# seungjunlee96/lightning-generative-models

Measured on AMD Instinct MI355X. Metric: training images/sec (DDPM UNet 32x32, bs=128), higher is better.
Workload: dtype f32; 1 GPU; configs/diffusion/ddpm.json UNet dim=64, 3x32x32 synthetic NCHW fp32, training_step+backward+Adam+EMA; global_batch=128, per_gpu_batch=128, parallelism=dp1, launch=hipGraph replay (1 graph/step)

## Files before the change

### lightning-generative-models_amd/csrc/linattn_fused.hip

```cpp
#include <type_traits>

#include "lgm_common.h"

namespace {

constexpr int DH = 32;
constexpr int HEADS = 4;
constexpr int HID = HEADS * DH;
constexpr int C = 64;
constexpr int LD = 36;
constexpr int TP = 128;
constexpr int XLD = 80;
constexpr int WLD = 100;

struct FArgs {
  const float* qkv;  long pitch;
  const float* gout; long gout_pitch;
  const float* ctx; const float* gctx; const float* kmax; const float* ksum; const float* rvec;
  const float* xn;   long xn_pitch;
  const float* wt;
  float* gxn;        long gxn_pitch;
  float* slabs;
  int n, tiles, items, per;
  float scale;
};

__device__ __forceinline__ void load16(const float* p, float (&v)[16]) {
#pragma unroll
  for (int q = 0; q < 4; ++q) {
    const f32x4 t = *reinterpret_cast<const f32x4*>(p + 4 * q);
    v[4 * q] = t[0]; v[4 * q + 1] = t[1]; v[4 * q + 2] = t[2]; v[4 * q + 3] = t[3];
  }
}

__global__ __launch_bounds__(256, 1) void linattn_bwd_fused_kernel(const FArgs p) {
  extern __shared__ __align__(16) float sm[];
  float* Qs = sm;
  float* Ks = Qs + TP * LD;
  float* Vs = Ks + TP * LD;
  float* Gs = Vs + TP * LD;
  float* Cs = Gs + TP * LD;
  float* GCs = Cs + DH * LD;
  float* GCt = GCs + DH * LD;
  float* rr = GCt + DH * LD;
  float* Ws = rr + DH;
  float* Xs = Ws + C * WLD;
  const int tid = threadIdx.x;
  const int lane = tid & 63, wid = tid >> 6;
  const int lr = lane & 31, lh = lane >> 5;
  const int l16 = lane & 15, lq = lane >> 4;
  const int c4 = (tid & 7) * 4, prow = tid >> 3;
  const int srow = 32 * wid + (lane >> 1), spart = (lane & 1) * 16;
  const int it0 = blockIdx.x * p.per, it1 = min(p.items, it0 + p.per);
  if (it0 >= it1) return;

  int w_src[6], w_dst[6];
#pragma unroll
  for (int u = 0; u < 6; ++u) {
    const int e = tid + 256 * u;
    const int c = e / 24, rem = e - 24 * c;
    const int part = rem >> 3, j = rem & 7;
    w_src[u] = c * (3 * HID) + part * HID + 4 * j;
    w_dst[u] = c * WLD + part * DH + 4 * j;
  }

  f32x4 q4[4], k4[4], v4[4], g4[4], km4, ks4, cx4, gc4, w4[6];
  float rr1 = 0.f;
  auto issue = [&](int it, int h) {
    const int b = it / p.tiles, i0 = (it % p.tiles) * TP;
    const int rows = min(TP, p.n - i0);
    const long bh = (long)b * HEADS + h;
#pragma unroll
    for (int u = 0; u < 4; ++u) {
      const int r = prow + 32 * u;
      const long row = (long)b * p.n + i0 + (r < rows ? r : 0);
      const float* qp = p.qkv + row * p.pitch + h * DH + c4;
      q4[u] = *reinterpret_cast<const f32x4*>(qp);
      k4[u] = *reinterpret_cast<const f32x4*>(qp + HID);
      v4[u] = *reinterpret_cast<const f32x4*>(qp + 2 * HID);
      g4[u] = *reinterpret_cast<const f32x4*>(p.gout + row * p.gout_pitch + h * DH + c4);
    }
    km4 = *reinterpret_cast<const f32x4*>(p.kmax + bh * DH + c4);
    ks4 = *reinterpret_cast<const f32x4*>(p.ksum + bh * DH + c4);
    cx4 = *reinterpret_cast<const f32x4*>(p.ctx + bh * DH * DH + tid * 4);
    gc4 = *reinterpret_cast<const f32x4*>(p.gctx + bh * DH * DH + tid * 4);
    if (tid < DH) rr1 = p.rvec[bh * DH + tid];
#pragma unroll
    for (int u = 0; u < 6; ++u) w4[u] = *reinterpret_cast<const f32x4*>(p.wt + w_src[u] + h * DH);
  };

  f32x4 dacc[HEADS][6];
#pragma unroll
  for (int h = 0; h < HEADS; ++h)
#pragma unroll
    for (int t = 0; t < 6; ++t) dacc[h][t] = f32x4{0.f, 0.f, 0.f, 0.f};
  const f32x4 zero4 = {0.f, 0.f, 0.f, 0.f};

  issue(it0, 0);
  for (int it = it0; it < it1; ++it) {
    const int b = it / p.tiles, i0 = (it % p.tiles) * TP;
    const int rows = min(TP, p.n - i0);
    f32x16 acc[2];
#pragma unroll
    for (int a = 0; a < 2; ++a)
#pragma unroll
      for (int r = 0; r < 16; ++r) acc[a][r] = 0.f;
    {
#pragma unroll
      for (int u = 0; u < 4; ++u) {
        const int r = prow + 32 * u;
        const long row = (long)b * p.n + i0 + (r < rows ? r : 0);
#pragma unroll
        for (int hf = 0; hf < 2; ++hf) {
          f32x4 xv = *reinterpret_cast<const f32x4*>(p.xn + row * p.xn_pitch + hf * 32 + c4);
          if (r >= rows) xv = zero4;
          *reinterpret_cast<f32x4*>(Xs + r * XLD + hf * 32 + c4) = xv;
        }
      }
    }
    auto head = [&](auto hc) {
      constexpr int h = decltype(hc)::value;
#pragma unroll
      for (int u = 0; u < 4; ++u) {
        const int r = prow + 32 * u;
        const bool live = r < rows;
        f32x4 kv;
#pragma unroll
        for (int k = 0; k < 4; ++k) kv[k] = __expf(k4[u][k] - km4[k]) * (1.f / ks4[k]);
        *reinterpret_cast<f32x4*>(Qs + r * LD + c4) = live ? q4[u] : zero4;
        *reinterpret_cast<f32x4*>(Ks + r * LD + c4) = live ? kv : zero4;
        *reinterpret_cast<f32x4*>(Vs + r * LD + c4) = live ? v4[u] : zero4;
        *reinterpret_cast<f32x4*>(Gs + r * LD + c4) = live ? g4[u] : zero4;
      }
      {
        const int d = tid >> 3, e0 = (tid & 7) * 4;
        *reinterpret_cast<f32x4*>(Cs + d * LD + e0) = cx4;
        *reinterpret_cast<f32x4*>(GCs + d * LD + e0) = gc4;
#pragma unroll
        for (int k = 0; k < 4; ++k) GCt[(e0 + k) * LD + d] = gc4[k];
      }
      if (tid < DH) rr[tid] = rr1;
#pragma unroll
      for (int u = 0; u < 6; ++u) *reinterpret_cast<f32x4*>(Ws + w_dst[u]) = w4[u];
      __syncthreads();
      if (h + 1 < HEADS) issue(it, h + 1);
      else if (it + 1 < it1) issue(it + 1, 0);

      float sv[16];
      {
        load16(Qs + srow * LD + spart, sv);
        float mx = sv[0];
#pragma unroll
        for (int k = 1; k < 16; ++k) mx = fmaxf(mx, sv[k]);
        mx = fmaxf(mx, __shfl_xor(mx, 1, 64));
        float sum = 0.f;
#pragma unroll
        for (int k = 0; k < 16; ++k) {
          sv[k] = __expf(sv[k] - mx);
          sum += sv[k];
        }
        sum += __shfl_xor(sum, 1, 64);
        const float inv = 1.f / sum;
#pragma unroll
        for (int k = 0; k < 16; ++k) sv[k] *= inv;
      }
      f32x16 a1, a2, a3;
#pragma unroll
      for (int r = 0; r < 16; ++r) a1[r] = a2[r] = a3[r] = 0.f;
      {
        float ca[16], ga[16], ta[16], gb[16], vb[16], kb[16];
        load16(Cs + lr * LD + 16 * lh, ca);
        load16(GCs + lr * LD + 16 * lh, ga);
        load16(GCt + lr * LD + 16 * lh, ta);
        load16(Gs + (32 * wid + lr) * LD + 16 * lh, gb);
        load16(Vs + (32 * wid + lr) * LD + 16 * lh, vb);
        load16(Ks + (32 * wid + lr) * LD + 16 * lh, kb);
#pragma unroll
        for (int s = 0; s < 16; ++s) {
          a1 = __builtin_amdgcn_mfma_f32_32x32x2f32(ca[s], gb[s], a1, 0, 0, 0);
          a2 = __builtin_amdgcn_mfma_f32_32x32x2f32(ga[s], vb[s], a2, 0, 0, 0);
          a3 = __builtin_amdgcn_mfma_f32_32x32x2f32(ta[s], kb[s], a3, 0, 0, 0);
        }
      }
      lgm_wave_lds_sync();
      {
        float* gp = Gs + (32 * wid + lr) * LD + 4 * lh;
        float* vp = Vs + (32 * wid + lr) * LD + 4 * lh;
#pragma unroll
        for (int g = 0; g < 4; ++g) {
          *reinterpret_cast<f32x4*>(gp + 8 * g) = f32x4{a1[4 * g], a1[4 * g + 1], a1[4 * g + 2], a1[4 * g + 3]};
          *reinterpret_cast<f32x4*>(vp + 8 * g) = f32x4{a2[4 * g], a2[4 * g + 1], a2[4 * g + 2], a2[4 * g + 3]};
        }
      }
      lgm_wave_lds_sync();
      {
        float g1[16], t2[16], kk[16], rv[16], dot = 0.f;
        load16(Gs + srow * LD + spart, g1);
        load16(Vs + srow * LD + spart, t2);
        load16(Ks + srow * LD + spart, kk);
        load16(rr + spart, rv);
#pragma unroll
        for (int k = 0; k < 16; ++k) {
          g1[k] *= p.scale;
          dot += sv[k] * g1[k];
        }
        dot += __shfl_xor(dot, 1, 64);
#pragma unroll
        for (int q = 0; q < 4; ++q) {
          f32x4 oq, ok;
#pragma unroll
          for (int k = 0; k < 4; ++k) {
            oq[k] = sv[4 * q + k] * (g1[4 * q + k] - dot);
            ok[k] = kk[4 * q + k] * (t2[4 * q + k] - rv[4 * q + k]);
          }
          *reinterpret_cast<f32x4*>(Qs + srow * LD + spart + 4 * q) = oq;
          *reinterpret_cast<f32x4*>(Ks + srow * LD + spart + 4 * q) = ok;
        }
      }
      lgm_wave_lds_sync();
      {
        float* vp = Vs + (32 * wid + lr) * LD + 4 * lh;
#pragma unroll
        for (int g = 0; g < 4; ++g)
          *reinterpret_cast<f32x4*>(vp + 8 * g) = f32x4{a3[4 * g], a3[4 * g + 1], a3[4 * g + 2], a3[4 * g + 3]};
      }
      lgm_wave_lds_sync();
#pragma unroll
      for (int part = 0; part < 3; ++part) {
        float xb[16], w0[16], w1[16];
        load16((part == 0 ? Qs : part == 1 ? Ks : Vs) + (32 * wid + lr) * LD + 16 * lh, xb);
        load16(Ws + lr * WLD + part * DH + 16 * lh, w0);
        load16(Ws + (32 + lr) * WLD + part * DH + 16 * lh, w1);
#pragma unroll
        for (int s = 0; s < 16; ++s) {
          acc[0] = __builtin_amdgcn_mfma_f32_32x32x2f32(w0[s], xb[s], acc[0], 0, 0, 0);
          acc[1] = __builtin_amdgcn_mfma_f32_32x32x2f32(w1[s], xb[s], acc[1], 0, 0, 0);
        }
      }
      __syncthreads();
      {
        const float* xb = Xs + lq * XLD + 16 * wid + l16;
#pragma unroll 4
        for (int s = 0; s < TP / 4; ++s) {
          const float bv = xb[4 * s * XLD];
#pragma unroll
          for (int part = 0; part < 3; ++part) {
            const float* X = (part == 0 ? Qs : part == 1 ? Ks : Vs) + (4 * s + lq) * LD + l16;
            dacc[h][2 * part] = __builtin_amdgcn_mfma_f32_16x16x4f32(X[0], bv, dacc[h][2 * part], 0, 0, 0);
            dacc[h][2 * part + 1] = __builtin_amdgcn_mfma_f32_16x16x4f32(X[16], bv, dacc[h][2 * part + 1], 0, 0, 0);
          }
        }
        __syncthreads();
      }
    };
    head(std::integral_constant<int, 0>{});
    head(std::integral_constant<int, 1>{});
    head(std::integral_constant<int, 2>{});
    head(std::integral_constant<int, 3>{});
    if (32 * wid + lr < rows) {
      float* o = p.gxn + ((long)b * p.n + i0 + 32 * wid + lr) * p.gxn_pitch + 4 * lh;
#pragma unroll
      for (int a = 0; a < 2; ++a)
#pragma unroll
        for (int g = 0; g < 4; ++g)
          *reinterpret_cast<f32x4*>(o + 32 * a + 8 * g) = f32x4{acc[a][4 * g], acc[a][4 * g + 1], acc[a][4 * g + 2], acc[a][4 * g + 3]};
    }
  }
  {
    float* sl = p.slabs + (long)blockIdx.x * (3 * HID * C);
#pragma unroll
    for (int h = 0; h < HEADS; ++h)
#pragma unroll
      for (int t = 0; t < 6; ++t)
#pragma unroll
        for (int r = 0; r < 4; ++r) {
          const int wrow = (t >> 1) * HID + h * DH + (t & 1) * 16 + 4 * lq + r;
          sl[(long)wrow * C + 16 * wid + l16] = dacc[h][t][r];
        }
  }
}

constexpr size_t kSmem = ((size_t)4 * TP * LD + 3 * DH * LD + DH + C * WLD + TP * XLD) * sizeof(float);

int plan_blocks(int B, int n, int* tiles, int* items, int* per) {
  *tiles = lgm_cdiv(n, TP);
  *items = B * *tiles;
  const int nb = *items < 256 ? *items : 256;
  *per = lgm_cdiv(*items, nb);
  return lgm_cdiv(*items, *per);
}

}

extern "C" int64_t lgm_linattn_bwd_fused_supported(int heads, int dim_head, int Cin) {
  return heads == HEADS && dim_head == DH && Cin == C ? 1 : 0;
}

extern "C" int64_t lgm_linattn_bwd_fused_slabs(int B, int n, int Cin) {
  if (Cin != C) return 0;
  int tiles, items, per;
  const int blocks = plan_blocks(B, n, &tiles, &items, &per);
  return (int64_t)blocks * 3 * HID * C * (int64_t)sizeof(float);
}

int lgm_linattn_bwd_fused_launch(const float* qkv, long pitch, const float* gout, long gout_pitch, const float* ctx,
                                 const float* gctx, const float* kmax, const float* ksum, const float* rvec,
                                 const float* xn, long xn_pitch, const float* wt, int B, int n, float scale,
                                 float* gxn, long gxn_pitch, float* slabs, int* blocks_out, hipStream_t s) {
  FArgs a;
  a.qkv = qkv; a.pitch = pitch; a.gout = gout; a.gout_pitch = gout_pitch;
  a.ctx = ctx; a.gctx = gctx; a.kmax = kmax; a.ksum = ksum; a.rvec = rvec;
  a.xn = xn; a.xn_pitch = xn_pitch; a.wt = wt; a.gxn = gxn; a.gxn_pitch = gxn_pitch;
  a.slabs = slabs; a.n = n; a.scale = scale;
  const int blocks = plan_blocks(B, n, &a.tiles, &a.items, &a.per);
  *blocks_out = blocks;
  lgm_note_kernel(LGM_KNAME("linattn_bwd_fused_kernel"));
  static bool attr = false;
  if (!attr) {
    (void)hipFuncSetAttribute(reinterpret_cast<const void*>(linattn_bwd_fused_kernel),
                              hipFuncAttributeMaxDynamicSharedMemorySize, (int)kSmem);
    attr = true;
  }
  hipLaunchKernelGGL(linattn_bwd_fused_kernel, dim3(blocks), dim3(256), kSmem, s, a);
  LGM_LAUNCH_CHECK();
  return LGM_OK;
}

namespace {

constexpr int OTP = 128;
constexpr int ALD = 132;

struct OArgs {
  const float* qkv;  long pitch;
  const float* ctx;
  const float* wout; const float* bout; const float* g;
  const float* x;    long x_pitch;
  float* ao;         long ao_pitch;
  float* o2;         long o2_pitch;
  float* y;          long y_pitch;
  int n, tiles, items, per;
  float scale;
};

template <int NC>
__global__ __launch_bounds__(256, NC == 2 ? 3 : 1) void linattn_out_fused_kernel(const OArgs p) {
  constexpr int CO = 32 * NC;
  extern __shared__ __align__(16) float sm[];
  float* Ws = sm;
  float* Ct = Ws + CO * ALD;
  const int tid = threadIdx.x;
  const int lane = tid & 63, wid = tid >> 6;
  const int lr = lane & 31, lh = lane >> 5;
  const int it0 = blockIdx.x * p.per, it1 = min(p.items, it0 + p.per);
  if (it0 >= it1) return;
  const float sqrtc = sqrtf((float)CO);

  f32x4 qn[4];
  auto issue_q = [&](int it, int h) {
    const int b = it / p.tiles, i0 = (it % p.tiles) * OTP;
    const int pix = min(i0 + 32 * wid + lr, p.n - 1);
    const float* qp = p.qkv + ((long)b * p.n + pix) * p.pitch + h * DH + 16 * lh;
#pragma unroll
    for (int j = 0; j < 4; ++j) qn[j] = *reinterpret_cast<const f32x4*>(qp + 4 * j);
  };
  issue_q(it0, 0);
#pragma unroll
  for (int u = 0; u < NC * 4; ++u) {
    const int e = tid + 256 * u;
    const int c = e >> 5, k4 = (e & 31) * 4;
    *reinterpret_cast<f32x4*>(Ws + c * ALD + k4) = *reinterpret_cast<const f32x4*>(p.wout + (long)c * HID + k4);
  }
  int b_staged = -1;
  for (int it = it0; it < it1; ++it) {
    const int b = it / p.tiles, i0 = (it % p.tiles) * OTP;
    const int pix = i0 + 32 * wid + lr;
    const bool live = pix < p.n;
    const long row = (long)b * p.n + min(pix, p.n - 1);
    if (b != b_staged) {
      __syncthreads();
#pragma unroll
      for (int u = 0; u < 4; ++u) {
        const int e = (tid + 256 * u) * 4;
        const int h = e >> 10, d = (e >> 5) & 31, e0 = e & 31;
        const f32x4 cv = *reinterpret_cast<const f32x4*>(p.ctx + (long)b * HEADS * DH * DH + e);
#pragma unroll
        for (int k = 0; k < 4; ++k) Ct[h * (DH * LD) + (e0 + k) * LD + d] = cv[k];
      }
      __syncthreads();
      b_staged = b;
    }
    f32x4 xres[NC <= 4 ? NC * 4 : 1];
    if constexpr (NC <= 4) {
#pragma unroll
      for (int a = 0; a < NC; ++a)
#pragma unroll
        for (int g = 0; g < 4; ++g)
          xres[a * 4 + g] = *reinterpret_cast<const f32x4*>(p.x + row * p.x_pitch + a * 32 + 8 * g + 4 * lh);
    }
    f32x16 acc[NC];
#pragma unroll
    for (int a = 0; a < NC; ++a)
#pragma unroll
      for (int r = 0; r < 16; ++r) acc[a][r] = 0.f;
#pragma unroll
    for (int h = 0; h < HEADS; ++h) {
      float qs[16];
#pragma unroll
      for (int j = 0; j < 4; ++j) {
        qs[4 * j] = qn[j][0]; qs[4 * j + 1] = qn[j][1]; qs[4 * j + 2] = qn[j][2]; qs[4 * j + 3] = qn[j][3];
      }
      if (h + 1 < HEADS) issue_q(it, h + 1);
      else if (it + 1 < it1) issue_q(it + 1, 0);
      float mx = qs[0];
#pragma unroll
      for (int k = 1; k < 16; ++k) mx = fmaxf(mx, qs[k]);
      mx = fmaxf(mx, __shfl_xor(mx, 32, 64));
      float sum = 0.f;
#pragma unroll
      for (int k = 0; k < 16; ++k) {
        qs[k] = __expf(qs[k] - mx);
        sum += qs[k];
      }
      sum += __shfl_xor(sum, 32, 64);
      const float inv = p.scale / sum;
      float ca[16];
      load16(Ct + h * (DH * LD) + lr * LD + 16 * lh, ca);
      f32x16 o;
#pragma unroll
      for (int r = 0; r < 16; ++r) o[r] = 0.f;
#pragma unroll
      for (int s = 0; s < 16; ++s) o = __builtin_amdgcn_mfma_f32_32x32x2f32(ca[s], qs[s] * inv, o, 0, 0, 0);
      if (live) {
#pragma unroll
        for (int g = 0; g < 4; ++g)
          *reinterpret_cast<f32x4*>(p.ao + row * p.ao_pitch + h * DH + 8 * g + 4 * lh) =
              f32x4{o[4 * g], o[4 * g + 1], o[4 * g + 2], o[4 * g + 3]};
      }
#pragma unroll
      for (int a = 0; a < NC; ++a) {
        const float* wp = Ws + (a * 32 + lr) * ALD + h * DH + 4 * lh;
#pragma unroll
        for (int g = 0; g < 4; ++g) {
          const f32x4 wv = *reinterpret_cast<const f32x4*>(wp + 8 * g);
#pragma unroll
          for (int j = 0; j < 4; ++j) acc[a] = __builtin_amdgcn_mfma_f32_32x32x2f32(wv[j], o[4 * g + j], acc[a], 0, 0, 0);
        }
      }
    }
    float ss = 0.f;
#pragma unroll
    for (int a = 0; a < NC; ++a)
#pragma unroll
      for (int g = 0; g < 4; ++g) {
        const f32x4 bv = *reinterpret_cast<const f32x4*>(p.bout + a * 32 + 8 * g + 4 * lh);
#pragma unroll
        for (int k = 0; k < 4; ++k) {
          acc[a][4 * g + k] += bv[k];
          ss += acc[a][4 * g + k] * acc[a][4 * g + k];
        }
      }
    ss += __shfl_xor(ss, 32, 64);
    const float rinv = sqrtc / fmaxf(sqrtf(ss), 1e-12f);
    if (live) {
#pragma unroll
      for (int a = 0; a < NC; ++a)
#pragma unroll
        for (int g = 0; g < 4; ++g) {
          const int c = a * 32 + 8 * g + 4 * lh;
          const f32x4 v = {acc[a][4 * g], acc[a][4 * g + 1], acc[a][4 * g + 2], acc[a][4 * g + 3]};
          const f32x4 gv = *reinterpret_cast<const f32x4*>(p.g + c);
          f32x4 xv;
          if constexpr (NC <= 4) xv = xres[a * 4 + g];
          else xv = *reinterpret_cast<const f32x4*>(p.x + row * p.x_pitch + c);
          *reinterpret_cast<f32x4*>(p.o2 + row * p.o2_pitch + c) = v;
          *reinterpret_cast<f32x4*>(p.y + row * p.y_pitch + c) = v * gv * rinv + xv;
        }
    }
  }
}

template <int NC>
int launch_out(const OArgs& a, int blocks, hipStream_t s) {
  const size_t smem = ((size_t)32 * NC * ALD + HEADS * DH * LD) * sizeof(float);
  static bool attr = false;
  if (!attr) {
    (void)hipFuncSetAttribute(reinterpret_cast<const void*>(linattn_out_fused_kernel<NC>),
                              hipFuncAttributeMaxDynamicSharedMemorySize, (int)smem);
    attr = true;
  }
  hipLaunchKernelGGL(linattn_out_fused_kernel<NC>, dim3(blocks), dim3(256), smem, s, a);
  LGM_LAUNCH_CHECK();
  return LGM_OK;
}

}

extern "C" int64_t lgm_linattn_fwd_fused_supported(int heads, int dim_head, int Cout) {
  if (heads != HEADS || dim_head != DH) return 0;
  return Cout == 64 || Cout == 128 ? 2 : Cout == 256 ? 1 : 0;
}

int lgm_linattn_out_fused_launch(const float* qkv, long pitch, const float* ctx, const float* wout, const float* bout,
                                 const float* g, const float* x, long x_pitch, float* ao, long ao_pitch, float* o2,
                                 long o2_pitch, float* y, long y_pitch, int B, int n, int Cout, float scale, hipStream_t s) {
  OArgs a;
  a.qkv = qkv; a.pitch = pitch; a.ctx = ctx; a.wout = wout; a.bout = bout; a.g = g; a.x = x; a.x_pitch = x_pitch;
  a.ao = ao; a.ao_pitch = ao_pitch; a.o2 = o2; a.o2_pitch = o2_pitch; a.y = y; a.y_pitch = y_pitch;
  a.n = n; a.scale = scale;
  a.tiles = lgm_cdiv(n, OTP);
  a.items = B * a.tiles;
  const int slots = Cout == 64 ? 768 : 256;
  const int nb = a.items < slots ? a.items : slots;
  a.per = lgm_cdiv(a.items, nb);
  const int blocks = lgm_cdiv(a.items, a.per);
  lgm_note_kernel(Cout == 64 ? LGM_KNAME("linattn_out_fused_kernel<2>") : Cout == 128 ? LGM_KNAME("linattn_out_fused_kernel<4>")
                                                                             : LGM_KNAME("linattn_out_fused_kernel<8>"));
  if (Cout == 64) return launch_out<2>(a, blocks, s);
  if (Cout == 128) return launch_out<4>(a, blocks, s);
  return launch_out<8>(a, blocks, s);
}

namespace {

struct QArgs {
  const float* x;  long x_pitch;
  const float* g;
  const float* w;
  float* xn;       long xn_pitch;
  float* qkv;      long q_pitch;
  long P;
  int items, per;
};

template <int NCI>
__global__ __launch_bounds__(256, NCI == 2 ? 3 : NCI == 4 ? 2 : 1) void rms_qkv_fused_kernel(const QArgs p) {
  constexpr int CI = 32 * NCI;
  constexpr int WL = CI + 4;
  extern __shared__ __align__(16) float sm[];
  float* Ws = sm;
  const int tid = threadIdx.x;
  const int lane = tid & 63, wid = tid >> 6;
  const int lr = lane & 31, lh = lane >> 5;
  int blk, slice;
  {
    const int nblk = (int)gridDim.x / 3, bid = (int)blockIdx.x;
    if (nblk % 8 == 0) {
      const int xcd = bid & 7, slot = bid >> 3;
      blk = (slot / 3) * 8 + xcd;
      slice = slot % 3;
    } else {
      blk = bid / 3;
      slice = bid % 3;
    }
  }
  const int it0 = blk * p.per, it1 = min(p.items, it0 + p.per);
  if (it0 >= it1) return;
  const float sqrtc = sqrtf((float)CI);
  f32x4 xr[NCI * 4];
  auto issue_x = [&](int it) {
    const long pix = (long)it * 128 + 32 * wid + lr;
    const long row = pix < p.P ? pix : p.P - 1;
#pragma unroll
    for (int a = 0; a < NCI; ++a)
#pragma unroll
      for (int g = 0; g < 4; ++g)
        xr[a * 4 + g] = *reinterpret_cast<const f32x4*>(p.x + row * p.x_pitch + a * 32 + 8 * g + 4 * lh);
  };
  issue_x(it0);
#pragma unroll
  for (int u = 0; u < NCI * 4; ++u) {
    const int e = tid + 256 * u;
    const int r = e / (CI / 4), c4 = (e % (CI / 4)) * 4;
    *reinterpret_cast<f32x4*>(Ws + r * WL + c4) = *reinterpret_cast<const f32x4*>(p.w + (long)(slice * 128 + r) * CI + c4);
  }
  __syncthreads();
  for (int it = it0; it < it1; ++it) {
    const long pix = (long)it * 128 + 32 * wid + lr;
    const bool live = pix < p.P;
    const long row = live ? pix : p.P - 1;
    f32x4 xn[NCI * 4];
    float ss = 0.f;
#pragma unroll
    for (int k = 0; k < NCI * 4; ++k) {
      xn[k] = xr[k];
      ss += xn[k][0] * xn[k][0] + xn[k][1] * xn[k][1] + xn[k][2] * xn[k][2] + xn[k][3] * xn[k][3];
    }
    if (NCI <= 4 && it + 1 < it1) issue_x(it + 1);
    ss += __shfl_xor(ss, 32, 64);
    const float inv = sqrtc / fmaxf(sqrtf(ss), 1e-12f);
#pragma unroll
    for (int a = 0; a < NCI; ++a)
#pragma unroll
      for (int g = 0; g < 4; ++g) {
        const f32x4 gv = *reinterpret_cast<const f32x4*>(p.g + a * 32 + 8 * g + 4 * lh);
        xn[a * 4 + g] = xn[a * 4 + g] * gv * inv;
        if (slice == 0 && live)
          *reinterpret_cast<f32x4*>(p.xn + row * p.xn_pitch + a * 32 + 8 * g + 4 * lh) = xn[a * 4 + g];
      }
#pragma unroll 1
    for (int t = 0; t < 4; ++t) {
      f32x16 acc;
#pragma unroll
      for (int r = 0; r < 16; ++r) acc[r] = 0.f;
      const float* wp = Ws + (t * 32 + lr) * WL + 4 * lh;
#pragma unroll
      for (int a = 0; a < NCI; ++a)
#pragma unroll
        for (int g = 0; g < 4; ++g) {
          const f32x4 wv = *reinterpret_cast<const f32x4*>(wp + a * 32 + 8 * g);
#pragma unroll
          for (int j = 0; j < 4; ++j) acc = __builtin_amdgcn_mfma_f32_32x32x2f32(wv[j], xn[a * 4 + g][j], acc, 0, 0, 0);
        }
      if (live) {
        float* o = p.qkv + row * p.q_pitch + slice * 128 + t * 32 + 4 * lh;
#pragma unroll
        for (int g = 0; g < 4; ++g)
          *reinterpret_cast<f32x4*>(o + 8 * g) = f32x4{acc[4 * g], acc[4 * g + 1], acc[4 * g + 2], acc[4 * g + 3]};
      }
    }
    if (NCI > 4 && it + 1 < it1) issue_x(it + 1);
  }
}

template <int NCI>
int launch_qkv(const QArgs& a, int blocks, hipStream_t s) {
  const size_t smem = (size_t)128 * (32 * NCI + 4) * sizeof(float);
  static bool attr = false;
  if (!attr) {
    (void)hipFuncSetAttribute(reinterpret_cast<const void*>(rms_qkv_fused_kernel<NCI>),
                              hipFuncAttributeMaxDynamicSharedMemorySize, (int)smem);
    attr = true;
  }
  hipLaunchKernelGGL(rms_qkv_fused_kernel<NCI>, dim3(blocks * 3), dim3(256), smem, s, a);
  LGM_LAUNCH_CHECK();
  return LGM_OK;
}

}

extern "C" int64_t lgm_rms_qkv_fused_supported(int C, int N) {
  if (N != 3 * HID) return 0;
  return C == 64 ? 2 : C == 128 || C == 256 ? 1 : 0;
}

extern "C" int lgm_rms_qkv_fused(const float* x, int64_t x_pitch, const float* g, const float* w, int C, int N,
                                 int64_t npix, float* xn, int64_t xn_pitch, float* qkv, int64_t qkv_pitch, void* stream) {
  LGM_REQUIRE(lgm_rms_qkv_fused_supported(C, N), "rms_qkv_fused: C=%d N=%d unsupported", C, N);
  LGM_REQUIRE(x && g && w && xn && qkv && npix > 0, "rms_qkv_fused: null pointer / empty");
  LGM_REQUIRE(x_pitch % 4 == 0 && xn_pitch % 4 == 0 && qkv_pitch % 4 == 0 && lgm_aligned16(x) && lgm_aligned16(g) &&
                  lgm_aligned16(w) && lgm_aligned16(xn) && lgm_aligned16(qkv),
              "rms_qkv_fused: 16-byte aligned operands required");
  QArgs a;
  a.x = x; a.x_pitch = x_pitch; a.g = g; a.w = w; a.xn = xn; a.xn_pitch = xn_pitch; a.qkv = qkv; a.q_pitch = qkv_pitch;
  a.P = npix;
  a.items = lgm_cdiv(npix, 128);
  const int slots = C == 64 ? 256 : C == 128 ? 170 : 85;
  const int nb = a.items < slots ? a.items : slots;
  a.per = lgm_cdiv(a.items, nb);
  const int blocks = lgm_cdiv(a.items, a.per);
  lgm_note_kernel(C == 64 ? LGM_KNAME("rms_qkv_fused_kernel<2>") : C == 128 ? LGM_KNAME("rms_qkv_fused_kernel<4>") : LGM_KNAME("rms_qkv_fused_kernel<8>"));
  hipStream_t s = (hipStream_t)stream;
  if (C == 64) return launch_qkv<2>(a, blocks, s);
  if (C == 128) return launch_qkv<4>(a, blocks, s);
  return launch_qkv<8>(a, blocks, s);
}
```

Baseline: 13680 images/s.

## Run fused linear-attention backward with 512 threads and 16x16 MFMA tiles

Measured after the change: 13780 images/s (median of 6 runs). No clear change (+0.8%).

```diff
diff --git a/lightning-generative-models_amd/csrc/linattn_fused.hip b/lightning-generative-models_amd/csrc/linattn_fused.hip
--- a/lightning-generative-models_amd/csrc/linattn_fused.hip
+++ b/lightning-generative-models_amd/csrc/linattn_fused.hip
@@ -10,7 +10,8 @@
 constexpr int C = 64;
 constexpr int LD = 36;
 constexpr int TP = 128;
-constexpr int XLD = 80;
+constexpr int BT = 512;
+constexpr int XLD = 68;
 constexpr int WLD = 100;
 
 struct FArgs {
@@ -33,7 +34,15 @@
   }
 }
 
-__global__ __launch_bounds__(256, 1) void linattn_bwd_fused_kernel(const FArgs p) {
+__device__ __forceinline__ void load8(const float* p, float (&v)[8]) {
+#pragma unroll
+  for (int q = 0; q < 2; ++q) {
+    const f32x4 t = *reinterpret_cast<const f32x4*>(p + 4 * q);
+    v[4 * q] = t[0]; v[4 * q + 1] = t[1]; v[4 * q + 2] = t[2]; v[4 * q + 3] = t[3];
+  }
+}
+
+__global__ __launch_bounds__(BT, 2) void linattn_bwd_fused_kernel(const FArgs p) {
   extern __shared__ __align__(16) float sm[];
   float* Qs = sm;
   float* Ks = Qs + TP * LD;
@@ -47,82 +56,81 @@
   float* Xs = Ws + C * WLD;
   const int tid = threadIdx.x;
   const int lane = tid & 63, wid = tid >> 6;
-  const int lr = lane & 31, lh = lane >> 5;
   const int l16 = lane & 15, lq = lane >> 4;
   const int c4 = (tid & 7) * 4, prow = tid >> 3;
-  const int srow = 32 * wid + (lane >> 1), spart = (lane & 1) * 16;
+  const int own = (16 * wid + l16) * LD + 8 * lq;
+  const int owd = (16 * wid + l16) * LD + 4 * lq;
+  const int ecg = wid & 3, erh = wid >> 2;
   const int it0 = blockIdx.x * p.per, it1 = min(p.items, it0 + p.per);
   if (it0 >= it1) return;
 
-  int w_src[6], w_dst[6];
-#pragma unroll
-  for (int u = 0; u < 6; ++u) {
-    const int e = tid + 256 * u;
-    const int c = e / 24, rem = e - 24 * c;
-    const int part = rem >> 3, j = rem & 7;
-    w_src[u] = c * (3 * HID) + part * HID + 4 * j;
-    w_dst[u] = c * WLD + part * DH + 4 * j;
-  }
-
-  f32x4 q4[4], k4[4], v4[4], g4[4], km4, ks4, cx4, gc4, w4[6];
+  const float* w_src = p.wt + prow * (3 * HID) + c4;
+  const int w_dst = prow * WLD + c4;
+
+  f32x4 q4[2], k4[2], v4[2], g4[2], km4, ks4, cg4, w4[3];
   float rr1 = 0.f;
   auto issue = [&](int it, int h) {
     const int b = it / p.tiles, i0 = (it % p.tiles) * TP;
     const int rows = min(TP, p.n - i0);
     const long bh = (long)b * HEADS + h;
-#pragma unroll
-    for (int u = 0; u < 4; ++u) {
-      const int r = prow + 32 * u;
-      const long row = (long)b * p.n + i0 + (r < rows ? r : 0);
-      const float* qp = p.qkv + row * p.pitch + h * DH + c4;
+    const float* qb = p.qkv + ((long)b * p.n + i0) * p.pitch + h * DH;
+    const float* gb = p.gout + ((long)b * p.n + i0) * p.gout_pitch + h * DH;
+#pragma unroll
+    for (int u = 0; u < 2; ++u) {
+      const int r = prow + 64 * u, rc = r < rows ? r : 0;
+      const float* qp = qb + (unsigned)(rc * (int)p.pitch + c4);
       q4[u] = *reinterpret_cast<const f32x4*>(qp);
       k4[u] = *reinterpret_cast<const f32x4*>(qp + HID);
       v4[u] = *reinterpret_cast<const f32x4*>(qp + 2 * HID);
-      g4[u] = *reinterpret_cast<const f32x4*>(p.gout + row * p.gout_pitch + h * DH + c4);
+      g4[u] = *reinterpret_cast<const f32x4*>(gb + (unsigned)(rc * (int)p.gout_pitch + c4));
     }
     km4 = *reinterpret_cast<const f32x4*>(p.kmax + bh * DH + c4);
     ks4 = *reinterpret_cast<const f32x4*>(p.ksum + bh * DH + c4);
-    cx4 = *reinterpret_cast<const f32x4*>(p.ctx + bh * DH * DH + tid * 4);
-    gc4 = *reinterpret_cast<const f32x4*>(p.gctx + bh * DH * DH + tid * 4);
+    cg4 = *reinterpret_cast<const f32x4*>((tid < 256 ? p.ctx : p.gctx) + bh * DH * DH + (tid & 255) * 4);
     if (tid < DH) rr1 = p.rvec[bh * DH + tid];
 #pragma unroll
-    for (int u = 0; u < 6; ++u) w4[u] = *reinterpret_cast<const f32x4*>(p.wt + w_src[u] + h * DH);
+    for (int u = 0; u < 3; ++u) w4[u] = *reinterpret_cast<const f32x4*>(w_src + u * HID + h * DH);
   };
 
-  f32x4 dacc[HEADS][6];
+  const f32x4 zero4 = {0.f, 0.f, 0.f, 0.f};
+  f32x4 dacc[HEADS][3];
 #pragma unroll
   for (int h = 0; h < HEADS; ++h)
 #pragma unroll
-    for (int t = 0; t < 6; ++t) dacc[h][t] = f32x4{0.f, 0.f, 0.f, 0.f};
-  const f32x4 zero4 = {0.f, 0.f, 0.f, 0.f};
+    for (int t = 0; t < 3; ++t) dacc[h][t] = zero4;
+
+  f32x4 xr[4];
+  auto issue_xn = [&](int it) {
+    const int b = it / p.tiles, i0 = (it % p.tiles) * TP;
+    const int rows = min(TP, p.n - i0);
+#pragma unroll
+    for (int u = 0; u < 2; ++u) {
+      const int r = prow + 64 * u, rc = r < rows ? r : 0;
+      const float* xp = p.xn + ((long)b * p.n + i0) * p.xn_pitch + (unsigned)(rc * (int)p.xn_pitch + c4);
+      xr[2 * u] = *reinterpret_cast<const f32x4*>(xp);
+      xr[2 * u + 1] = *reinterpret_cast<const f32x4*>(xp + 32);
+    }
+  };
 
   issue(it0, 0);
+  issue_xn(it0);
   for (int it = it0; it < it1; ++it) {
     const int b = it / p.tiles, i0 = (it % p.tiles) * TP;
     const int rows = min(TP, p.n - i0);
-    f32x16 acc[2];
-#pragma unroll
-    for (int a = 0; a < 2; ++a)
-#pragma unroll
-      for (int r = 0; r < 16; ++r) acc[a][r] = 0.f;
-    {
-#pragma unroll
-      for (int u = 0; u < 4; ++u) {
-        const int r = prow + 32 * u;
-        const long row = (long)b * p.n + i0 + (r < rows ? r : 0);
-#pragma unroll
-        for (int hf = 0; hf < 2; ++hf) {
-          f32x4 xv = *reinterpret_cast<const f32x4*>(p.xn + row * p.xn_pitch + hf * 32 + c4);
-          if (r >= rows) xv = zero4;
-          *reinterpret_cast<f32x4*>(Xs + r * XLD + hf * 32 + c4) = xv;
-        }
-      }
+    f32x4 acc[4];
+#pragma unroll
+    for (int t = 0; t < 4; ++t) acc[t] = zero4;
+#pragma unroll
+    for (int u = 0; u < 2; ++u) {
+      const int r = prow + 64 * u;
+      *reinterpret_cast<f32x4*>(Xs + r * XLD + c4) = r < rows ? xr[2 * u] : zero4;
+      *reinterpret_cast<f32x4*>(Xs + r * XLD + 32 + c4) = r < rows ? xr[2 * u + 1] : zero4;
     }
     auto head = [&](auto hc) {
       constexpr int h = decltype(hc)::value;
 #pragma unroll
-      for (int u = 0; u < 4; ++u) {
-        const int r = prow + 32 * u;
+      for (int u = 0; u < 2; ++u) {
+        const int r = prow + 64 * u;
         const bool live = r < rows;
         f32x4 kv;
 #pragma unroll
@@ -133,122 +141,141 @@
         *reinterpret_cast<f32x4*>(Gs + r * LD + c4) = live ? g4[u] : zero4;
       }
       {
-        const int d = tid >> 3, e0 = (tid & 7) * 4;
-        *reinterpret_cast<f32x4*>(Cs + d * LD + e0) = cx4;
-        *reinterpret_cast<f32x4*>(GCs + d * LD + e0) = gc4;
-#pragma unroll
-        for (int k = 0; k < 4; ++k) GCt[(e0 + k) * LD + d] = gc4[k];
+        const int d = prow & 31, e0 = c4;
+        if (tid < 256) {
+          *reinterpret_cast<f32x4*>(Cs + d * LD + e0) = cg4;
+        } else {
+          *reinterpret_cast<f32x4*>(GCs + d * LD + e0) = cg4;
+#pragma unroll
+          for (int k = 0; k < 4; ++k) GCt[(e0 + k) * LD + d] = cg4[k];
+        }
       }
       if (tid < DH) rr[tid] = rr1;
 #pragma unroll
-      for (int u = 0; u < 6; ++u) *reinterpret_cast<f32x4*>(Ws + w_dst[u]) = w4[u];
+      for (int u = 0; u < 3; ++u) *reinterpret_cast<f32x4*>(Ws + w_dst + u * DH) = w4[u];
       __syncthreads();
       if (h + 1 < HEADS) issue(it, h + 1);
       else if (it + 1 < it1) issue(it + 1, 0);
 
-      float sv[16];
+      float sv[8];
       {
-        load16(Qs + srow * LD + spart, sv);
+        load8(Qs + own, sv);
         float mx = sv[0];
 #pragma unroll
-        for (int k = 1; k < 16; ++k) mx = fmaxf(mx, sv[k]);
-        mx = fmaxf(mx, __shfl_xor(mx, 1, 64));
+        for (int k = 1; k < 8; ++k) mx = fmaxf(mx, sv[k]);
+        mx = fmaxf(mx, __shfl_xor(mx, 16, 64));
+        mx = fmaxf(mx, __shfl_xor(mx, 32, 64));
         float sum = 0.f;
 #pragma unroll
-        for (int k = 0; k < 16; ++k) {
+        for (int k = 0; k < 8; ++k) {
           sv[k] = __expf(sv[k] - mx);
           sum += sv[k];
         }
-        sum += __shfl_xor(sum, 1, 64);
+        sum += __shfl_xor(sum, 16, 64);
+        sum += __shfl_xor(sum, 32, 64);
         const float inv = 1.f / sum;
 #pragma unroll
-        for (int k = 0; k < 16; ++k) sv[k] *= inv;
-      }
-      f32x16 a1, a2, a3;
-#pragma unroll
-      for (int r = 0; r < 16; ++r) a1[r] = a2[r] = a3[r] = 0.f;
+        for (int k = 0; k < 8; ++k) sv[k] *= inv;
+      }
+      f32x4 a1[2], a2[2], a3[2];
       {
-        float ca[16], ga[16], ta[16], gb[16], vb[16], kb[16];
-        load16(Cs + lr * LD + 16 * lh, ca);
-        load16(GCs + lr * LD + 16 * lh, ga);
-        load16(GCt + lr * LD + 16 * lh, ta);
-        load16(Gs + (32 * wid + lr) * LD + 16 * lh, gb);
-        load16(Vs + (32 * wid + lr) * LD + 16 * lh, vb);
-        load16(Ks + (32 * wid + lr) * LD + 16 * lh, kb);
-#pragma unroll
-        for (int s = 0; s < 16; ++s) {
-          a1 = __builtin_amdgcn_mfma_f32_32x32x2f32(ca[s], gb[s], a1, 0, 0, 0);
-          a2 = __builtin_amdgcn_mfma_f32_32x32x2f32(ga[s], vb[s], a2, 0, 0, 0);
-          a3 = __builtin_amdgcn_mfma_f32_32x32x2f32(ta[s], kb[s], a3, 0, 0, 0);
-        }
+        float gb[8], vb[8], kb[8];
+        load8(Gs + own, gb);
+        load8(Vs + own, vb);
+        load8(Ks + own, kb);
+#pragma unroll
+        for (int t = 0; t < 2; ++t) {
+          float ca[8], ga[8], ta[8];
+          load8(Cs + (16 * t + l16) * LD + 8 * lq, ca);
+          load8(GCs + (16 * t + l16) * LD + 8 * lq, ga);
+          load8(GCt + (16 * t + l16) * LD + 8 * lq, ta);
+          a1[t] = a2[t] = a3[t] = zero4;
+#pragma unroll
+          for (int s = 0; s < 8; ++s) {
+            a1[t] = __builtin_amdgcn_mfma_f32_16x16x4f32(ca[s], gb[s], a1[t], 0, 0, 0);
+            a2[t] = __builtin_amdgcn_mfma_f32_16x16x4f32(ga[s], vb[s], a2[t], 0, 0, 0);
+            a3[t] = __builtin_amdgcn_mfma_f32_16x16x4f32(ta[s], kb[s], a3[t], 0, 0, 0);
+          }
+        }
+      }
+      lgm_wave_lds_sync();
+#pragma unroll
+      for (int t = 0; t < 2; ++t) {
+        *reinterpret_cast<f32x4*>(Gs + owd + 16 * t) = a1[t];
+        *reinterpret_cast<f32x4*>(Vs + owd + 16 * t) = a2[t];
       }
       lgm_wave_lds_sync();
       {
-        float* gp = Gs + (32 * wid + lr) * LD + 4 * lh;
-        float* vp = Vs + (32 * wid + lr) * LD + 4 * lh;
-#pragma unroll
-        for (int g = 0; g < 4; ++g) {
-          *reinterpret_cast<f32x4*>(gp + 8 * g) = f32x4{a1[4 * g], a1[4 * g + 1], a1[4 * g + 2], a1[4 * g + 3]};
-          *reinterpret_cast<f32x4*>(vp + 8 * g) = f32x4{a2[4 * g], a2[4 * g + 1], a2[4 * g + 2], a2[4 * g + 3]};
-        }
-      }
-      lgm_wave_lds_sync();
-      {
-        float g1[16], t2[16], kk[16], rv[16], dot = 0.f;
-        load16(Gs + srow * LD + spart, g1);
-        load16(Vs + srow * LD + spart, t2);
-        load16(Ks + srow * LD + spart, kk);
-        load16(rr + spart, rv);
-#pragma unroll
-        for (int k = 0; k < 16; ++k) {
+        float g1[8], t2[8], kk[8], rv[8], dot = 0.f;
+        load8(Gs + own, g1);
+        load8(Vs + own, t2);
+        load8(Ks + own, kk);
+        load8(rr + 8 * lq, rv);
+#pragma unroll
+        for (int k = 0; k < 8; ++k) {
           g1[k] *= p.scale;
           dot += sv[k] * g1[k];
         }
-        dot += __shfl_xor(dot, 1, 64);
-#pragma unroll
-        for (int q = 0; q < 4; ++q) {
+        dot += __shfl_xor(dot, 16, 64);
+        dot += __shfl_xor(dot, 32, 64);
+#pragma unroll
+        for (int q = 0; q < 2; ++q) {
           f32x4 oq, ok;
 #pragma unroll
           for (int k = 0; k < 4; ++k) {
             oq[k] = sv[4 * q + k] * (g1[4 * q + k] - dot);
             ok[k] = kk[4 * q + k] * (t2[4 * q + k] - rv[4 * q + k]);
           }
-          *reinterpret_cast<f32x4*>(Qs + srow * LD + spart + 4 * q) = oq;
-          *reinterpret_cast<f32x4*>(Ks + srow * LD + spart + 4 * q) = ok;
+          *reinterpret_cast<f32x4*>(Qs + own + 4 * q) = oq;
+          *reinterpret_cast<f32x4*>(Ks + own + 4 * q) = ok;
         }
       }
       lgm_wave_lds_sync();
+#pragma unroll
+      for (int t = 0; t < 2; ++t) *reinterpret_cast<f32x4*>(Vs + owd + 16 * t) = a3[t];
+      lgm_wave_lds_sync();
+#pragma unroll
+      for (int part = 0; part < 3; ++part) {
+        float xb[8];
+        load8((part == 0 ? Qs : part == 1 ? Ks : Vs) + own, xb);
+#pragma unroll
+        for (int t = 0; t < 4; ++t) {
+          float wv[8];
+          load8(Ws + (16 * t + l16) * WLD + part * DH + 8 * lq, wv);
+#pragma unroll
+          for (int s = 0; s < 8; ++s) acc[t] = __builtin_amdgcn_mfma_f32_16x16x4f32(wv[s], xb[s], acc[t], 0, 0, 0);
+        }
+      }
+      __syncthreads();
+      if (h + 1 == HEADS && it + 1 < it1) issue_xn(it + 1);
       {
-        float* vp = Vs + (32 * wid + lr) * LD + 4 * lh;
-#pragma unroll
-        for (int g = 0; g < 4; ++g)
-          *reinterpret_cast<f32x4*>(vp + 8 * g) = f32x4{a3[4 * g], a3[4 * g + 1], a3[4 * g + 2], a3[4 * g + 3]};
-      }
-      lgm_wave_lds_sync();
-#pragma unroll
-      for (int part = 0; part < 3; ++part) {
-        float xb[16], w0[16], w1[16];
-        load16((part == 0 ? Qs : part == 1 ? Ks : Vs) + (32 * wid + lr) * LD + 16 * lh, xb);
-        load16(Ws + lr * WLD + part * DH + 16 * lh, w0);
-        load16(Ws + (32 + lr) * WLD + part * DH + 16 * lh, w1);
-#pragma unroll
-        for (int s = 0; s < 16; ++s) {
-          acc[0] = __builtin_amdgcn_mfma_f32_32x32x2f32(w0[s], xb[s], acc[0], 0, 0, 0);
-          acc[1] = __builtin_amdgcn_mfma_f32_32x32x2f32(w1[s], xb[s], acc[1], 0, 0, 0);
-        }
-      }
-      __syncthreads();
-      {
-        const float* xb = Xs + lq * XLD + 16 * wid + l16;
-#pragma unroll 4
-        for (int s = 0; s < TP / 4; ++s) {
-          const float bv = xb[4 * s * XLD];
-#pragma unroll
-          for (int part = 0; part < 3; ++part) {
-            const float* X = (part == 0 ? Qs : part == 1 ? Ks : Vs) + (4 * s + lq) * LD + l16;
-            dacc[h][2 * part] = __builtin_amdgcn_mfma_f32_16x16x4f32(X[0], bv, dacc[h][2 * part], 0, 0, 0);
-            dacc[h][2 * part + 1] = __builtin_amdgcn_mfma_f32_16x16x4f32(X[16], bv, dacc[h][2 * part + 1], 0, 0, 0);
+        const float* xb = Xs + 4 * lq * XLD + 16 * ecg + l16;
+        const int xo = 4 * lq * LD + 16 * erh + l16;
+        float eb[2][4], eq[2][4], ek[2][4], ev[2][4];
+        auto fetch = [&](int g, int set) {
+#pragma unroll
+          for (int j = 0; j < 4; ++j) {
+            eb[set][j] = xb[(16 * g + j) * XLD];
+            eq[set][j] = Qs[(16 * g + j) * LD + xo];
+            ek[set][j] = Ks[(16 * g + j) * LD + xo];
+            ev[set][j] = Vs[(16 * g + j) * LD + xo];
           }
+        };
+        auto mult = [&](int set) {
+#pragma unroll
+          for (int j = 0; j < 4; ++j) {
+            dacc[h][0] = __builtin_amdgcn_mfma_f32_16x16x4f32(eq[set][j], eb[set][j], dacc[h][0], 0, 0, 0);
+            dacc[h][1] = __builtin_amdgcn_mfma_f32_16x16x4f32(ek[set][j], eb[set][j], dacc[h][1], 0, 0, 0);
+            dacc[h][2] = __builtin_amdgcn_mfma_f32_16x16x4f32(ev[set][j], eb[set][j], dacc[h][2], 0, 0, 0);
+          }
+        };
+        fetch(0, 0);
+#pragma unroll 1
+        for (int g = 0; g < TP / 16; g += 2) {
+          fetch(g + 1, 1);
+          mult(0);
+          if (g + 2 < TP / 16) fetch(g + 2, 0);
+          mult(1);
         }
         __syncthreads();
       }
@@ -257,13 +284,10 @@
     head(std::integral_constant<int, 1>{});
     head(std::integral_constant<int, 2>{});
     head(std::integral_constant<int, 3>{});
-    if (32 * wid + lr < rows) {
-      float* o = p.gxn + ((long)b * p.n + i0 + 32 * wid + lr) * p.gxn_pitch + 4 * lh;
-#pragma unroll
-      for (int a = 0; a < 2; ++a)
-#pragma unroll
-        for (int g = 0; g < 4; ++g)
-          *reinterpret_cast<f32x4*>(o + 32 * a + 8 * g) = f32x4{acc[a][4 * g], acc[a][4 * g + 1], acc[a][4 * g + 2], acc[a][4 * g + 3]};
+    if (16 * wid + l16 < rows) {
+      float* o = p.gxn + ((long)b * p.n + i0 + 16 * wid + l16) * p.gxn_pitch + 4 * lq;
+#pragma unroll
+      for (int t = 0; t < 4; ++t) *reinterpret_cast<f32x4*>(o + 16 * t) = acc[t];
     }
   }
   {
@@ -271,11 +295,11 @@
 #pragma unroll
     for (int h = 0; h < HEADS; ++h)
 #pragma unroll
-      for (int t = 0; t < 6; ++t)
+      for (int part = 0; part < 3; ++part)
 #pragma unroll
         for (int r = 0; r < 4; ++r) {
-          const int wrow = (t >> 1) * HID + h * DH + (t & 1) * 16 + 4 * lq + r;
-          sl[(long)wrow * C + 16 * wid + l16] = dacc[h][t][r];
+          const int wrow = part * HID + h * DH + 16 * erh + 4 * lq + r;
+          sl[(long)wrow * C + 16 * ecg + l16] = dacc[h][part][r];
         }
   }
 }
@@ -321,7 +345,7 @@
                               hipFuncAttributeMaxDynamicSharedMemorySize, (int)kSmem);
     attr = true;
   }
-  hipLaunchKernelGGL(linattn_bwd_fused_kernel, dim3(blocks), dim3(256), kSmem, s, a);
+  hipLaunchKernelGGL(linattn_bwd_fused_kernel, dim3(blocks), dim3(BT), kSmem, s, a);
   LGM_LAUNCH_CHECK();
   return LGM_OK;
 }
```
